# wendazhou/nbodyhpc

Hardware: AMD Instinct MI355X
Metric: kNN queries/sec (k=32, 1e8 periodic particles) (higher is better)
Workload: dtype f32; 1 GPU; kNN k=32 self-query of every particle, 1e+08 uniform periodic particles (L=1.0), leafsize 64; n_particles=100000000, n_particles_per_gpu=100000000, k=32, leafsize=64, parallelism=single

## Files before the change

### include/nbkd.h

```cpp
#ifndef NBKD_H
#define NBKD_H

#include <stdint.h>

#ifdef __cplusplus
extern "C" {
#endif

typedef int32_t nbkd_status;

enum {
    NBKD_OK = 0,
    NBKD_EINVAL = 1,
    NBKD_EBOX = 2,
    NBKD_ETOOMANY = 3,
    NBKD_ENOMEM = 4,
    NBKD_EDEVICE = 5,
    NBKD_EINTR = 6
};

#define NBKD_INPUT_DEVICE 0x1u
#define NBKD_OUTPUT_DEVICE 0x2u
#define NBKD_ACCUMULATE 0x4u
#define NBKD_SQUARED 0x8u
// ... 74 lines not shown
                               uint32_t flags, void *stream);

nbkd_status nbkd_group_potential(const nbkd_tree *tree,
                                 const uint64_t *offsets, const uint32_t *members,
                                 uint64_t ngroups, uint64_t nmembers,
                                 const float *mass, float eps, uint32_t max_members,
                                 float *out_phi, uint32_t *out_minpos,
                                 uint32_t flags, void *stream);

nbkd_status nbkd_query_ball_csr(const nbkd_tree *tree, const float *q, uint64_t m, float r,
                                uint64_t *out_offsets, uint32_t *out_idx, uint64_t capacity,
                                uint32_t flags, void *stream);

nbkd_status nbkd_tree_info(const nbkd_tree *tree, uint64_t *n8, uint64_t *nodes,
                           int32_t *periodic, float *box_size, int32_t *device);

nbkd_status nbkd_export(const nbkd_tree *tree, nbkd_node *nodes, float *x, float *y, float *z,
                        uint32_t *idx);

void nbkd_free(nbkd_tree *tree);

nbkd_status nbkd_set_tuning(const char *name, double value);
nbkd_status nbkd_get_tuning(const char *name, double *value);

typedef int (*nbkd_interrupt_fn)(void *user);
nbkd_status nbkd_set_interrupt(nbkd_interrupt_fn fn, void *user);

const char *nbkd_last_error(void);

nbkd_status nbkd_device_count(int32_t *count);

nbkd_status nbkd_timing_enable(int32_t enable);
nbkd_status nbkd_timing_reset(void);
nbkd_status nbkd_timing_read(const char *name, double *ms, uint64_t *launches);

nbkd_status nbkd_stats_enable(int32_t enable);
nbkd_status nbkd_stats_read(uint64_t *nodes_visited, uint64_t *points_scanned);
nbkd_status nbkd_stats_read_all(uint64_t *out, int32_t n);


nbkd_status nbkd_set_ids(nbkd_tree *tree, const uint32_t *ids, uint32_t flags, void *stream);

nbkd_status nbkd_set_kth_out(nbkd_tree *tree, float *kth, uint64_t capacity);

nbkd_status nbkd_slab_select(const float *xyz, const uint32_t *ids, uint64_t n, float lo, float hi,
                             float *out_xyz, uint32_t *out_ids, uint64_t capacity,
// ... 43 lines not shown
```

### nbodyhpc_amd/capi.py

```python
from __future__ import annotations

import ctypes
import os
import re

import numpy as np

PKG = os.path.dirname(os.path.abspath(__file__))
LIB_PATH = os.environ.get("NBKD_LIB") or os.path.join(PKG, "lib", "libnbkd.so")
HEADER = os.path.join(os.path.dirname(PKG), "include", "nbkd.h")

NBKD_OK, NBKD_EINVAL, NBKD_EBOX, NBKD_ETOOMANY, NBKD_ENOMEM, NBKD_EDEVICE, NBKD_EINTR = range(7)
NBKD_INPUT_DEVICE = 0x1
NBKD_OUTPUT_DEVICE = 0x2
NBKD_ACCUMULATE = 0x4
NBKD_SQUARED = 0x8
NBKD_SORTED = 0x10
KERNEL_TOPHAT, KERNEL_CUBIC, KERNEL_WENDLAND = 0, 1, 2
NBKD_MAX_VALUES = 4
NBKD_MAX_RADII = 32
NBKD_EWALD_N = 64

NODE_DTYPE = np.dtype([("dim", "<i4"), ("split", "<f4"), ("left", "<u4"), ("right", "<u4")])

# ... 44 lines not shown
    "nbkd_last_error": (ctypes.c_char_p, []),
    "nbkd_device_count": (_i32, [ctypes.POINTER(_i32)]),
    "nbkd_timing_enable": (_i32, [_i32]),
    "nbkd_timing_reset": (_i32, []),
    "nbkd_timing_read": (_i32, [ctypes.c_char_p, ctypes.POINTER(ctypes.c_double),
                                ctypes.POINTER(_u64)]),
    "nbkd_stats_enable": (_i32, [_i32]),
    "nbkd_stats_read": (_i32, [ctypes.POINTER(_u64), ctypes.POINTER(_u64)]),
    "nbkd_stats_read_all": (_i32, [ctypes.POINTER(_u64), _i32]),
    "nbkd_set_ids": (_i32, [_c_p, _c_p, _u32, _c_p]),
    "nbkd_slab_select": (_i32, [_c_p, _c_p, _u64, ctypes.c_float, ctypes.c_float, _c_p, _c_p,
                                _u64, ctypes.POINTER(_u64), _i32, _c_p]),
    "nbkd_slab_violations": (_i32, [_c_p, _c_p, _u64, _i32, ctypes.c_float, ctypes.c_float,
                                    ctypes.c_float, ctypes.POINTER(_u64), _i32, _c_p]),
    "nbkd_slab_forward": (_i32, [_c_p, _c_p, _u64, _i32, ctypes.c_float, ctypes.c_float, _c_p,
                                 _c_p, _u64, ctypes.POINTER(_u64), _i32, _c_p]),
    "nbkd_slab_forward_async": (_i32, [_c_p, _c_p, _u64, _i32, ctypes.c_float, ctypes.c_float,
                                       _c_p, _c_p, _u64, _c_p, _i32, _c_p]),
    "nbkd_rows_gather": (_i32, [_c_p, _u64, _c_p, _u64, _c_p, _i32, _c_p]),
    "nbkd_rows_scatter": (_i32, [_c_p, _u64, _c_p, _u64, _c_p, _i32, _c_p]),
    "nbkd_set_tuning": (_i32, [ctypes.c_char_p, ctypes.c_double]),
    "nbkd_set_interrupt": (_i32, [_c_p, _c_p]),
    "nbkd_get_tuning": (_i32, [ctypes.c_char_p, ctypes.POINTER(ctypes.c_double)]),
    "nbkd_comm_probe": (_i32, []),
    "nbkd_comm_unique_id": (_i32, [_c_p]),
    "nbkd_comm_init": (_i32, [_c_p, _i32, _i32, _i32, ctypes.POINTER(_c_p)]),
    "nbkd_comm_exchange": (_i32, [_c_p, _i32, _c_p, _c_p, _c_p, _c_p, _c_p, _c_p, _c_p]),
    "nbkd_comm_free": (None, [_c_p]),
    "nbkd_deposit": (_i32, [_c_p, _c_p, _c_p, _u64, _i32, _i32, _i32, ctypes.c_float, _c_p, _i32,
                            _i32, _i32, _i32, _c_p, _i32, _u32, _c_p]),
}
COMM_ID_BYTES = 128


def header_symbols() -> list[str]:
    txt = open(HEADER).read()
    txt = re.sub(r"/\*.*?\*/", "", txt, flags=re.S)
    return sorted(set(re.findall(r"\b(nbkd_[a-z_]+)\s*\(", txt)))


_lib = None


def lib():
    global _lib
    if _lib is None:
# ... 376 lines not shown
    flags = NBKD_INPUT_DEVICE | NBKD_OUTPUT_DEVICE | (NBKD_ACCUMULATE if accumulate else 0)
    _check(lib().nbkd_deposit(xyz_ptr, weight_ptr, radius_ptr, int(n), gx, gy, nz, float(ppu),
                              per.ctypes.data, int(subsample), int(mode), x0, wx, out_ptr,
                              int(device), flags, stream))


def ewald_table():
    nn = NBKD_EWALD_N + 1
    out = np.empty((nn, nn, nn, 4), np.float32)
    _check(lib().nbkd_ewald_table(out.ctypes.data, out.size))
    return out


def set_tuning(name, value):
    _check(lib().nbkd_set_tuning(name.encode(), float(value)))


def get_tuning(name):
    v = ctypes.c_double()
    _check(lib().nbkd_get_tuning(name.encode(), ctypes.byref(v)))
    return v.value


def timing_enable(on=True):
    _check(lib().nbkd_timing_enable(1 if on else 0))


def timing_reset():
    _check(lib().nbkd_timing_reset())


def timing_read(name):
    ms, cnt = ctypes.c_double(), _u64()
    _check(lib().nbkd_timing_read(name.encode(), ctypes.byref(ms), ctypes.byref(cnt)))
    return ms.value, cnt.value


def stats_enable(on=True):
    _check(lib().nbkd_stats_enable(1 if on else 0))


def stats_read():
    a, b = _u64(), _u64()
    _check(lib().nbkd_stats_read(ctypes.byref(a), ctypes.byref(b)))
    return a.value, b.value

# ... 100 lines not shown
```

### nbodyhpc_amd/csrc/api.cpp

```cpp
#include <hip/hip_runtime.h>

#include <sched.h>

#include <atomic>
#include <cmath>
#include <condition_variable>
#include <cstdio>
#include <cstring>
#include <map>
#include <mutex>
#include <new>
#include <string>
#include <thread>
#include <vector>

#include "internal.hpp"

namespace nbkd {

namespace {
thread_local std::string g_err;
thread_local uint64_t g_stats[NBKD_NSTATS] = {};

std::mutex g_tmu;
// ... 212 lines not shown
}

void tree_free(void *p) {
    if (!p) return;
    BlockCache &c = block_cache();
    std::lock_guard<std::mutex> g(c.mu);
    auto it = c.live.find(p);
    if (it == c.live.end()) {
        (void)hipFree(p);
        return;
    }
    const auto key = it->second;
    c.live.erase(it);
    if (c.idle_bytes + key.second <= BlockCache::CAP) {
        c.idle.insert({key, p});
        c.idle_bytes += key.second;
    } else {
        (void)hipFree(p);
    }
}


namespace {
std::atomic<double> g_tune[TUNE_N] = {{3.0}, {0.0}, {0.0}, {0.0}, {1.0}, {0.0}};
const char *const g_tune_names[TUNE_N] = {"knn_seed_margin", "candidate_bytes", "host_batch",
                                          "host_threads", "self_order", "pinned_bytes"};
thread_local nbkd_interrupt_fn t_intr = nullptr;
thread_local void *t_intr_user = nullptr;
}

double tuning(int id) { return g_tune[id].load(std::memory_order_relaxed); }

bool interrupted() { return t_intr != nullptr && t_intr(t_intr_user) != 0; }

Workspace &acquire_ws(const Tree &t) {
    if (t.ws.mu.try_lock()) return t.ws;
    {
        std::lock_guard<std::mutex> g(t.ws_mu);
        for (auto &w : t.ws_extra)
            if (w->mu.try_lock()) return *w;
        if ((int)t.ws_extra.size() < NBKD_MAX_WS - 1) {
            t.ws_extra.emplace_back(new Workspace());
            Workspace &w = *t.ws_extra.back();
            w.mu.lock();
            return w;
        }
    }
    t.ws.mu.lock();
    return t.ws;
// ... 703 lines not shown
    delete tree;
}

nbkd_status nbkd_set_tuning(const char *name, double value) {
    if (!name) {
        set_error("nbkd_set_tuning: NULL name");
        return NBKD_EINVAL;
    }
    for (int i = 0; i < TUNE_N; ++i) {
        if (std::strcmp(name, g_tune_names[i]) != 0) continue;
        const bool ok = i == TUNE_KNN_SEED ? (value > 0.0 && value <= 1e3)
                                           : (value >= 0.0 && value < 1e15);
        if (!ok || !std::isfinite(value)) {
            set_error(std::string("nbkd_set_tuning: value out of range for ") + name);
            return NBKD_EINVAL;
        }
        g_tune[i].store(value, std::memory_order_relaxed);
        return NBKD_OK;
    }
    set_error(std::string("nbkd_set_tuning: unknown knob ") + name);
    return NBKD_EINVAL;
}

nbkd_status nbkd_get_tuning(const char *name, double *value) {
    if (!name || !value) {
        set_error("nbkd_get_tuning: NULL argument");
        return NBKD_EINVAL;
    }
    for (int i = 0; i < TUNE_N; ++i)
        if (std::strcmp(name, g_tune_names[i]) == 0) {
            *value = tuning(i);
            return NBKD_OK;
        }
    set_error(std::string("nbkd_get_tuning: unknown knob ") + name);
    return NBKD_EINVAL;
}

nbkd_status nbkd_set_interrupt(nbkd_interrupt_fn fn, void *user) {
    t_intr = fn;
    t_intr_user = user;
    return NBKD_OK;
}

nbkd_status nbkd_timing_enable(int32_t enable) {
    g_timing = enable != 0;
    return NBKD_OK;
// ... 191 lines not shown
```

### nbodyhpc_amd/csrc/internal.hpp

```cpp
#pragma once

#include <hip/hip_runtime.h>

#include <cfloat>
#include <cstdint>
#include <cstdlib>
#include <memory>
#include <mutex>
#include <string>
#include <vector>

#include "../../include/nbkd.h"

namespace nbkd {

enum WsSlot {
    WS_Q = 0, WS_KEYS, WS_KEYS2, WS_ORDER, WS_TMP, WS_HIST, WS_SUMS, WS_OUTD, WS_OUTI,
    WS_COUNT, WS_OFF, WS_IDX, WS_STATS, WS_LIST, WS_LT, WS_TG, WS_CAND, WS_CCOUNT,
    WS_LIST2, WS_RSORT, WS_KTHD, WS_KTHI, WS_KB, WS_ANCH, WS_PAIR, WS_HTOT,
    WS_VT, WS_VALS, WS_HRAD,
    WS_GRAV,
    WS_HQ0, WS_HQ1, WS_HO00, WS_HO01, WS_HO10, WS_HO11, WS_NSLOTS
};
constexpr int NBKD_MAX_WS = 4;
// ... 116 lines not shown
    uint32_t n8;
    uint32_t nnodes;
    float box;
    const float *__restrict__ nbox;
};

inline DevTree view(const Tree &t) {
    return DevTree{t.x, t.y, t.z, t.idx, t.p4, t.nodes, (uint32_t)t.n8, (uint32_t)t.nnodes, t.box,
                   t.nbox};
}

#ifdef NBKD_EXPERIMENTS
inline const char *knob(const char *env) { return getenv(env); }
#else
inline const char *knob(const char *) { return nullptr; }
#endif
enum TuneId {
    TUNE_KNN_SEED = 0,
    TUNE_CAND_BYTES,
    TUNE_HOST_BATCH,
    TUNE_HOST_THREADS,
    TUNE_SELF_ORDER,
    TUNE_PINNED_BYTES,
    TUNE_N
};
void host_copy(void *dst, const void *src, size_t bytes);
int host_workers();
bool interrupted();
double tuning(int id);

void set_error(const std::string &msg);
nbkd_status hip_fail(hipError_t e, const char *what);

#define NBKD_HIP(call)                                                                     \
    do {                                                                                   \
        hipError_t e_ = (call);                                                            \
        if (e_ != hipSuccess) return ::nbkd::hip_fail(e_, #call);                          \
    } while (0)

struct TimedScope {
    TimedScope(const char *name, hipStream_t s, bool on = true);
    ~TimedScope();
    const char *name_;
    hipStream_t s_;
    hipEvent_t a_ = nullptr;
    int dev_ = 0;
// ... 33 lines not shown
nbkd_status build_tree(Tree &t, const float *xyz, uint64_t n, int32_t leaf_size, bool input_dev,
                       hipStream_t s);

struct QSpan {
    uint32_t m;
    const uint32_t *count;
    uint32_t base;
    uint32_t total;
    int mode;
    bool capped = false;
    bool tg_pos = false;
    uint32_t *out_list = nullptr;
    uint32_t *out_count = nullptr;
};
__host__ __device__ inline QSpan static_span(uint32_t m) { return QSpan{m, nullptr, 0u, 0u, 0}; }
__device__ __forceinline__ uint32_t span_m(const QSpan &s) {
    if (!s.count) return s.m;
    const uint32_t c = __builtin_amdgcn_readfirstlane(*s.count);
    if (s.mode != 0 && (((uint64_t)c * 512u >= (uint64_t)s.total) != (s.mode == 1))) return 0u;
    return c > s.base ? min(c - s.base, s.m) : 0u;
}

uint32_t collect_capacity(int k);
bool retry_adaptive();
nbkd_status launch_knn_collect(const Tree &t, const float *q, const uint32_t *order, QSpan span,
                               int k, const float *tg, float seed_mul, uint32_t qpp, uint2 *cand,
                               uint32_t capg, uint32_t *ccount, float *od, uint32_t *oi,
                               uint32_t *fail_list, uint32_t *fail_count, uint32_t *fail_bits,
                               uint32_t pos_base, bool retry, bool fix_seed, bool sq, float *kb,
                               unsigned long long *stats, hipStream_t s,
                               float *kth_side = nullptr, uint32_t *pair_scratch = nullptr);

nbkd_status launch_collect_pass(const Tree &t, const float *q, const uint32_t *order, QSpan span,
                                int k, const float *tg, float seed_mul, uint32_t qpp, uint2 *cand,
                                uint32_t capg, uint32_t *ccount, bool retry, float *kb,
                                unsigned long long *stats, hipStream_t s);
nbkd_status launch_select_pass(const Tree &t, const float *q, const uint32_t *order, QSpan span,
                               int k, const float *tg, uint32_t qpp, const uint2 *cand,
                               uint32_t capg, const uint32_t *ccount, float *od, uint32_t *oi,
                               uint32_t *fail_list, uint32_t *fail_count, uint32_t *fail_bits,
                               uint32_t pos_base, bool retry, bool fix_seed, bool sq, float *kb,
                               hipStream_t s, float *kth_side = nullptr,
                               uint32_t *pair_scratch = nullptr);

void launch_ball_packet(const Tree &t, const float *q, const uint32_t *order, uint32_t m, float r2,
                        uint32_t *out_count, const uint64_t *row_offsets, uint32_t *out_idx,
// ... 142 lines not shown
```

### nbodyhpc_amd/csrc/knn_collect.hip

```cpp
#include <algorithm>

#include "internal.hpp"
#include "metric.hpp"
#include "packet.hpp"

namespace nbkd {
namespace {
using namespace dev;

constexpr int TB = 256;
constexpr int WPB = TB / 64;

#ifndef NBKD_COL_ROWMAJOR
#define NBKD_COL_ROWMAJOR 1
#endif
#ifndef NBKD_PAIR_PAD
#define NBKD_PAIR_PAD 1
#endif
#ifndef NBKD_PAIR_ATOMIC
#define NBKD_PAIR_ATOMIC 1
#endif
#ifndef NBKD_SEL_FIRST
#define NBKD_SEL_FIRST 1
#endif
#ifndef NBKD_WAVE_KEY64
#define NBKD_WAVE_KEY64 1
#endif
#ifndef NBKD_WAVE_PAIR
#define NBKD_WAVE_PAIR 4
#endif
#ifndef NBKD_LOOP_AHEAD
#define NBKD_LOOP_AHEAD 1
#endif
#ifndef NBKD_RETRY_GROW
#define NBKD_RETRY_GROW 1.0f
#endif
#ifndef NBKD_RETRY_MINV
#define NBKD_RETRY_MINV 2.0f
#endif
#ifndef NBKD_SCL_EARLY
#define NBKD_SCL_EARLY 0
#endif
#ifndef NBKD_PAIR_PREFETCH
#define NBKD_PAIR_PREFETCH 0
#endif

constexpr int NB = 16;

__device__ __forceinline__ uint32_t d2_bucket(float d, float c) {
    return min((uint32_t)(d * c), (uint32_t)(NB - 1));
}


constexpr int GCHUNK = 64;
constexpr int GMAX = GCHUNK / NBKD_GROUP;

constexpr uint32_t PR_OWNER = NBKD_PAIR_PAD ? 7 : 6, PR_G = NBKD_PAIR_PAD ? 13 : 12;
constexpr uint32_t PR_SLOT = (1u << PR_OWNER) - 1u;
constexpr uint32_t PAIR_DUMMY = 64u;

struct CollectLdsG {
    float4 sq[64 + NBKD_PAIR_PAD];
    float scl[64];
    uint32_t cnt[64];
    uint32_t hist[NB / 4][65];
    float4 p4[GCHUNK];
    float gb[6 * GMAX];
    float tb[8];
    uint16_t pairs[64 * GMAX];
    uint8_t slot[64];
};

#define NBKD_COLLECT_STAGE_G(LPOS, CN, TBOX)                                                       \
    do {                                                                                           \
        glds_f4(t.p4 + (LPOS), W.p4, lane, (CN));                                                  \
        glds_f32(ginfo + 6 * (size_t)((LPOS) / NBKD_GROUP), W.gb, lane, 6 * ((CN) / NBKD_GROUP));  \
        glds_f32((TBOX), W.tb, lane, 6);                                                           \
    } while (0)

template <bool PER, bool M, bool STATS, bool AHEAD>
__device__ __forceinline__ void grp_packet(const DevTree &t, const float *__restrict__ ginfo,
                                           const uint32_t *__restrict__ linfo,
                                           const float *__restrict__ hinfo,
                                           CollectLdsG &W, const int lane, const float qx,
                                           const float qy, const float qz, float &kth,
                                           const float s_over_nb, const float nb_over_s,
                                           uint2 *__restrict__ col, const uint32_t qpp,
                                           const uint32_t capg, const int kq, uint32_t &cnt,
                                           uint32_t (&st)[13]) {
    const float L = t.box;
    uint32_t last_cnt = 0;
    const cnode_ptr cnodes = (cnode_ptr)t.nodes;
    const cbox_ptr cboxes = (cbox_ptr)t.nbox;
    PacketWalk wk;
    walk_begin(wk);
    uint64_t tclk = STATS ? clock64() : 0;
#define NBKD_PH(I)                                                                                 \
    do {                                                                                           \
        if constexpr (STATS) {                                                                     \
            const uint64_t t_ = clock64();                                                         \
            st[6 + (I)] += (uint32_t)(t_ - tclk);                                                              \
            tclk = t_;                                                                             \
        }                                                                                          \
    } while (0)
    bool ha = false;
    uint32_t pa = 0, ea = 0, lnode = 0;
    for (;;) {
        uint32_t pa_next = 0, ea_next = 0;
        const bool ha_next = walk_next_leaf<M, STATS>(wk, cnodes, cboxes, qx, qy, qz, kth, L, pa_next,
                                                      ea_next, st[0]);
        if constexpr (!AHEAD) {
            if (!ha_next) break;
            ha = true;
            pa = pa_next;
            ea = ea_next;
            lnode = wk.node;
        }
        if (ha) {
            const uint32_t lend = ea;
            const uint32_t lc = lend - pa;
            const bool halves = hinfo != nullptr && lc > (uint32_t)GCHUNK && lc <= 2u * GCHUNK;
            const uint32_t hm = (lc / 2) / 8 * 8;
            const float *const lbox = halves ? hinfo + 12 * (size_t)lnode
                                             : reinterpret_cast<const float *>(linfo) + 8 * (size_t)lnode;
            uint32_t c0 = pa;
            uint32_t cn = halves ? hm : min((uint32_t)GCHUNK, lc);
            if constexpr (!AHEAD) {
                if constexpr (STATS) ++st[3];
                NBKD_COLLECT_STAGE_G(pa, cn, lbox);
            }
            NBKD_PH(0);
            wait_vm0();
            wave_sync();
// ... 148 lines not shown
                wait_vm0();
                wave_sync();
            }
            wave_sync();
        }
        if constexpr (AHEAD) {
            if (!ha_next) break;
            ha = true;
            pa = pa_next;
            ea = ea_next;
            lnode = wk.node;
            if constexpr (STATS) ++st[3];
            const uint32_t lc = ea - pa;
            const bool halves = hinfo != nullptr && lc > (uint32_t)GCHUNK && lc <= 2u * GCHUNK;
            NBKD_COLLECT_STAGE_G(pa, halves ? (lc / 2) / 8 * 8 : min((uint32_t)GCHUNK, lc),
                                 halves ? hinfo + 12 * (size_t)lnode
                                        : reinterpret_cast<const float *>(linfo) + 8 * (size_t)lnode);
        }
    }
    NBKD_PH(0);
#undef NBKD_PH
}

template <bool PER, bool STATS, bool AHEAD>
__device__ __forceinline__ void collect_packet(
    const DevTree &t, const float *__restrict__ ginfo, const uint32_t *__restrict__ linfo,
    const float *__restrict__ hinfo, const float *__restrict__ q, const uint32_t *__restrict__ order,
    uint32_t m, int kq, const float *__restrict__ tg, bool tg_pos, float seed_mul, uint32_t qpp,
    uint2 *__restrict__ cand, uint32_t capg, uint32_t *__restrict__ ccount,
    unsigned long long *__restrict__ stats, float *__restrict__ kbound, CollectLdsG &W, int lane,
    uint32_t pk, uint32_t *__restrict__ out_list, uint32_t *__restrict__ out_count) {
    const uint32_t gq = pk * qpp + lane;
    const bool valid = (uint32_t)lane < qpp && gq < m;
    const uint32_t qo = valid ? order[gq] : 0u;
    const float qx = valid ? q[3 * (size_t)qo] : 0.0f;
    const float qy = valid ? q[3 * (size_t)qo + 1] : 0.0f;
    const float qz = valid ? q[3 * (size_t)qo + 2] : 0.0f;
    if constexpr (PER) {
        if (out_list && valid &&
            !(qx >= 0.0f && qx <= t.box && qy >= 0.0f && qy <= t.box && qz >= 0.0f && qz <= t.box))
            out_list[atomicAdd(out_count, 1u)] = qo;
    }
    const float seed = valid ? fminf(tg[tg_pos ? gq : qo] * seed_mul, FLT_MAX) : -INFINITY;
    const bool fin = seed < FLT_MAX && seed >= 1e-30f;
    const float s_over_nb = fin ? seed * (1.0f / NB) : (seed > 0.0f ? INFINITY : 0.0f);
    const float nb_over_s = fin ? (float)NB / seed * 1.00000095367431640625f : 0.0f;
#pragma unroll
    for (int w = 0; w < NB / 4; ++w) W.hist[w][lane] = 0u;
#if NBKD_PAIR_PAD
    if (lane == 0) W.sq[PAIR_DUMMY] = make_float4(0.0f, 0.0f, 0.0f, -INFINITY);
#endif
    uint2 *const col = cand + (size_t)pk * qpp * capg;
    uint32_t cnt = 0;
    uint32_t st[13] = {0, 0, 0, 0, 0, 0, 0, 0, 0, 0, 0, 0, 0};
    float kth = seed;
    bool plain = false;
    if constexpr (PER) {
        const float r1 = sqrtf(fmaxf(seed, 0.0f)) * 1.01f + t.box * 1e-6f;
        const bool wf = !valid || (fin && r1 <= 0.25f * t.box && qx >= r1 && t.box - qx >= r1 &&
                                   qy >= r1 && t.box - qy >= r1 && qz >= r1 && t.box - qz >= r1);
        plain = __all(wf);
    }
    if (plain)
        grp_packet<PER, false, STATS, AHEAD>(t, ginfo, linfo, hinfo, W, lane, qx, qy, qz, kth,
                                             s_over_nb, nb_over_s, col, qpp, capg, kq, cnt, st);
    else
        grp_packet<PER, PER, STATS, AHEAD>(t, ginfo, linfo, hinfo, W, lane, qx, qy, qz, kth,
                                           s_over_nb, nb_over_s, col, qpp, capg, kq, cnt, st);
    if (valid) ccount[gq] = cnt;
    if (valid && kbound) kbound[gq] = kth;
    if (STATS && lane == 0) {
        atomicAdd(&stats[0], (unsigned long long)st[0]);
        atomicAdd(&stats[1], (unsigned long long)st[5]);
        atomicAdd(&stats[2], (unsigned long long)st[3]);
        atomicAdd(&stats[3], (unsigned long long)st[4]);
        atomicAdd(&stats[4], (unsigned long long)st[2]);
        atomicAdd(&stats[5], 1ull);
        atomicAdd(&stats[7], (unsigned long long)st[1]);
#pragma unroll
        for (int i = 0; i < 6; ++i) atomicAdd(&stats[10 + i], (unsigned long long)st[6 + i]);
        atomicAdd(&stats[16], (unsigned long long)st[12]);
    }
    if (STATS) {
        uint32_t c = valid ? cnt : 0u;
#pragma unroll
        for (int o = 32; o > 0; o >>= 1) c += __shfl_xor(c, o, 64);
        if (lane == 0) atomicAdd(&stats[6], (unsigned long long)c);
    }
}

template <bool PER, int OCC, bool STATS, bool LOOP, bool AHEAD>
__global__ void __launch_bounds__(TB, OCC)
knn_collect_grp_kernel(DevTree t, const float *__restrict__ ginfo,
                       const uint32_t *__restrict__ linfo, const float *__restrict__ hinfo,
                       const float *__restrict__ q,
                       const uint32_t *__restrict__ order, QSpan span, int kq,
                       const float *__restrict__ tg, float seed_mul, uint32_t qpp,
                       uint2 *__restrict__ cand, uint32_t capg,
                       uint32_t *__restrict__ ccount, unsigned long long *__restrict__ stats,
                       bool xcd, float *__restrict__ kbound) {
    __shared__ CollectLdsG Wl[WPB];
    const int lane = threadIdx.x & 63, wave = wave_id();
    CollectLdsG &W = Wl[wave];
    const uint32_t m = span_m(span);
    const uint32_t npk = (m + qpp - 1) / qpp;
    const uint32_t bid = xcd ? xcd_block(blockIdx.x, gridDim.x) : blockIdx.x;
    if constexpr (LOOP) {
        for (uint32_t pk = bid * WPB + wave; pk < npk; pk += gridDim.x * WPB) {
            wave_sync();
            collect_packet<PER, STATS, AHEAD>(t, ginfo, linfo, hinfo, q, order, m, kq, tg, span.tg_pos,
                                              seed_mul, qpp, cand, capg, ccount, stats, kbound,
                                              W, lane, pk, span.out_list, span.out_count);
        }
    } else {
        const uint32_t pk = bid * WPB + wave;
        if (pk < npk)
            collect_packet<PER, STATS, AHEAD>(t, ginfo, linfo, hinfo, q, order, m, kq, tg, span.tg_pos,
                                              seed_mul, qpp, cand, capg, ccount, stats, kbound,
                                              W, lane, pk, span.out_list, span.out_count);
    }
}

template <bool PER>
__device__ __forceinline__ void mark_failure(float qx, float qy, float qz, float L, uint32_t id,
                                             uint32_t *fail_list, uint32_t *fail_count,
                                             uint32_t *fail_bits) {
    if (PER && !(qx >= 0.0f && qx <= L && qy >= 0.0f && qy <= L && qz >= 0.0f && qz <= L)) return;
    if (fail_bits)
        atomicOr(&fail_bits[id >> 5], 1u << (id & 31u));
    else
        fail_list[atomicAdd(fail_count, 1u)] = id;
}

__device__ __forceinline__ void issue_block(const uint4 *b4, uint4 *lds4, int lane, uint64_t rows,
                                            uint32_t row_stride4) {
    const uint32_t r0 = (uint32_t)lane >> 3, jj = (uint32_t)lane & 7u;
    const uint4 *src = b4 + r0 * row_stride4 + (jj ^ r0);
    const uint32_t m = (uint32_t)((((rows >> r0) & 0x0101010101010101ull) * 0x0102040810204080ull) >> 56);
#pragma unroll
    for (int i = 0; i < 8; ++i)
// ... 556 lines not shown
        return 8u * (unsigned)std::max(cus, 1);
    }();
    return b;
}

template <bool PER>
void launch_collect(const Tree &t, const float *q, const uint32_t *order, QSpan span, int k,
                    const float *tg, float seed_mul, uint32_t qpp, uint2 *cand, uint32_t capg,
                    uint32_t *ccount, unsigned long long *stats, bool retry, float *kbound,
                    hipStream_t s) {
    const char *const name = retry ? "knn_retry" : "knn_collect";
    const uint32_t m = span.m;
    const unsigned blocks =
        span.count ? std::min<unsigned>(resident_blocks(),
                                        (unsigned)((((uint64_t)m + qpp - 1) / qpp + WPB - 1) / WPB))
                   : (unsigned)((((uint64_t)m + qpp - 1) / qpp + WPB - 1) / WPB);
    if (k > 255) k = 0x7FFFFFFF;
    {
        static const bool xcd = [] {
            const char *e = knob("NBKD_XCD_MAP");
            return !(e && atoi(e) == 0);
        }();
        TimedScope ts(name, s, !retry);
#define NBKD_GRP(STATS, LOOP, AHEAD, STP, XCD)                                                     \
    knn_collect_grp_kernel<PER, 8, STATS, LOOP, AHEAD><<<blocks, TB, 0, s>>>(                      \
        view(t), t.ginfo, t.leafinfo, t.hinfo, q, order, span, k, tg, seed_mul, qpp, cand, capg,   \
        ccount, STP, XCD, kbound)
        if (span.count)
            NBKD_GRP(false, true, NBKD_LOOP_AHEAD != 0, nullptr, false);
        else if (collect_ahead()) {
            if (stats)
                NBKD_GRP(true, false, true, stats, xcd);
            else
                NBKD_GRP(false, false, true, nullptr, xcd);
        } else if (stats)
            NBKD_GRP(true, false, false, stats, xcd);
        else
            NBKD_GRP(false, false, false, nullptr, xcd);
#undef NBKD_GRP
        return;
    }
}

template <int R>
void launch_select_wave(const Tree &t, const float *q, const uint32_t *order, QSpan span, int k,
                        uint32_t qpp, const uint2 *cand, uint32_t capg, const uint32_t *ccount,
                        float *od, uint32_t *oi, uint32_t *fail_list, uint32_t *fail_count,
                        uint32_t *fail_bits, uint32_t pos_base, float *tg_fix, float mu, bool sq,
                        const float *kbound, hipStream_t s, uint32_t *pair_scratch) {
    const uint32_t *pos_list = nullptr;
    if constexpr (R == 2 && NBKD_COL_ROWMAJOR && NBKD_WAVE_PAIR > 0) {
        if (pair_scratch && !span.count && kbound) {
            uint32_t *nleft = pair_scratch + ((size_t)span.m + 15) / 16 * 16;
            if (hipMemsetAsync(nleft, 0, 4, s) != hipSuccess) goto one_query;
            {
            constexpr int NQ = NBKD_WAVE_PAIR;
            const unsigned pblocks = (unsigned)std::min<uint64_t>(
                (((uint64_t)span.m + NQ - 1) / NQ + WPB - 1) / WPB, 32768u);
            if (t.periodic)
                knn_select_wave_pair_kernel<true, NQ><<<pblocks, TB, 0, s>>>(
                    order, span, k, cand, capg, ccount, od, oi, sq, kbound, pair_scratch, nleft);
            else
// ... 48 lines not shown
        if (t.periodic) {
            if (qpp == 64) NBKD_SELECT(true, true, true); else NBKD_SELECT(true, false, true);
        } else {
            if (qpp == 64) NBKD_SELECT(false, true, true); else NBKD_SELECT(false, false, true);
        }
    } else {
        if (t.periodic) {
            if (qpp == 64) NBKD_SELECT(true, true, false); else NBKD_SELECT(true, false, false);
        } else {
            if (qpp == 64) NBKD_SELECT(false, true, false); else NBKD_SELECT(false, false, false);
        }
    }
#undef NBKD_SELECT
}

}

bool retry_adaptive() {
    static const bool on = [] {
        const char *e = knob("NBKD_RETRY_ADAPT");
        return !(e && atoi(e) == 0);
    }();
    return on;
}

uint32_t collect_capacity(int k) {
    const double mu = k + 4.0 * std::sqrt((double)k) + 4.0;
    double c = mu + 5.0 * std::sqrt(mu);
    if (const char *e = knob("NBKD_KNN_CAP")) c *= std::max(0.25, atof(e));
    return (uint32_t)((c + 15.0) / 16.0) * 16u;
}

nbkd_status launch_knn_collect(const Tree &t, const float *q, const uint32_t *order, QSpan span,
                               int k, const float *tg, float seed_mul, uint32_t qpp, uint2 *cand,
                               uint32_t capg, uint32_t *ccount, float *od, uint32_t *oi,
                               uint32_t *fail_list, uint32_t *fail_count, uint32_t *fail_bits,
                               uint32_t pos_base, bool retry, bool fix_seed, bool sq, float *kb,
                               unsigned long long *stats, hipStream_t s, float *kth_side,
                               uint32_t *pair_scratch) {
    nbkd_status rc = launch_collect_pass(t, q, order, span, k, tg, seed_mul, qpp, cand, capg,
                                         ccount, retry, kb, stats, s);
    if (rc) return rc;
    return launch_select_pass(t, q, order, span, k, tg, qpp, cand, capg, ccount, od, oi,
                              fail_list, fail_count, fail_bits, pos_base, retry, fix_seed, sq, kb,
                              s, kth_side, pair_scratch);
}
// ... 61 lines not shown
```

### nbodyhpc_amd/csrc/packet.hpp

```cpp
#pragma once

#include "metric.hpp"

namespace nbkd {
namespace dev {

typedef __attribute__((address_space(1))) const void *gas_ptr;
typedef __attribute__((address_space(3))) void *las_ptr;

__device__ __forceinline__ void glds_f32(const float *src, float *dst, int lane, uint32_t n) {
    if ((uint32_t)lane < n)
        __builtin_amdgcn_global_load_lds((gas_ptr)(src + lane), (las_ptr)dst, 4, 0, 0);
}

__device__ __forceinline__ void glds_f4(const float4 *src, float4 *dst, int lane, uint32_t n) {
    if ((uint32_t)lane < n)
        __builtin_amdgcn_global_load_lds((gas_ptr)(src + lane), (las_ptr)dst, 16, 0, 0);
}

__device__ __forceinline__ void wait_vm0() { __builtin_amdgcn_s_waitcnt(0x0F70); }

constexpr int pow2_floor(int v) { return v >= 64 ? 64 : v >= 32 ? 32 : v >= 16 ? 16 : v >= 8 ? 8 : 4; }
constexpr int pow2_ceil(int v) { return v <= 4 ? 4 : v <= 8 ? 8 : v <= 16 ? 16 : v <= 32 ? 32 : 64; }

// ... 150 lines not shown
        else                                                                                       \
            NBKD_GSTEP(2)                                                                          \
    }


struct PacketWalk {
    uint32_t node;
    int sp;
    uint32_t sk_node;
    uint32_t bx[6];
    float tm[3];
};

__device__ __forceinline__ void walk_begin(PacketWalk &w) {
    w.node = 0;
    w.sp = 1;
    w.sk_node = 0;
#pragma unroll
    for (int a = 0; a < 6; ++a) w.bx[a] = 0u;
#pragma unroll
    for (int a = 0; a < 3; ++a) w.tm[a] = 0.0f;
}

template <bool M>
__device__ __forceinline__ bool walk_step(PacketWalk &w, const int D, const uint32_t split_bits,
                                          const uint32_t left, const uint32_t right, uint64_t &wm,
                                          const float qx, const float qy, const float qz,
                                          const float kth, const float L) {
    const float split = __uint_as_float(split_bits);
    const float qd = D == 0 ? qx : (D == 1 ? qy : qz);
    float tl, tr;
    if constexpr (M) {
        const uint32_t lo = D == 0 ? w.bx[0] : (D == 1 ? w.bx[2] : w.bx[4]);
        const uint32_t hi = D == 0 ? w.bx[1] : (D == 1 ? w.bx[3] : w.bx[5]);
        tl = box_lb_axis<M>(qd, __uint_as_float(lo), split, L);
        tr = box_lb_axis<M>(qd, split, __uint_as_float(hi), L);
    } else {
        const float tmd = D == 0 ? w.tm[0] : (D == 1 ? w.tm[1] : w.tm[2]);
        const float dd = qd - split;
        const float m2 = dd * dd;
        tl = dd > 0.0f ? m2 : tmd;
        tr = dd > 0.0f ? tmd : m2;
    }
    const float dl = ((D == 0 ? tl : w.tm[0]) + (D == 1 ? tl : w.tm[1])) + (D == 2 ? tl : w.tm[2]);
    const float dr = ((D == 0 ? tr : w.tm[0]) + (D == 1 ? tr : w.tm[1])) + (D == 2 ? tr : w.tm[2]);
    const uint64_t wl = __ballot(dl <= kth), wr = __ballot(dr <= kth);
    bool go_right = wr != 0;
    if (wl != 0 && wr != 0) {
        const uint32_t right_votes = (uint32_t)__popcll(wm & __ballot(qd > split));
        go_right = 2 * right_votes > (uint32_t)__popcll(wm);
        w.sk_node = lane_set(w.sk_node, go_right ? left : right, 1ull << w.sp);
        ++w.sp;
    }
    w.node = go_right ? right : left;
    const float tn = go_right ? tr : tl;
    w.tm[0] = D == 0 ? tn : w.tm[0];
    w.tm[1] = D == 1 ? tn : w.tm[1];
    w.tm[2] = D == 2 ? tn : w.tm[2];
#pragma unroll
    for (int a = 0; a < 3; ++a) {
        w.bx[2 * a] = (D == a && go_right) ? split_bits : w.bx[2 * a];
        w.bx[2 * a + 1] = (D == a && !go_right) ? split_bits : w.bx[2 * a + 1];
    }
    wm = go_right ? wr : wl;
    return (wl | wr) != 0;
}

template <bool M, bool STATS>
__device__ __forceinline__ bool walk_next_leaf(PacketWalk &w, const cnode_ptr cnodes,
                                               const cbox_ptr cboxes, const float qx,
                                               const float qy, const float qz, const float kth,
                                               const float L, uint32_t &lpos, uint32_t &lend,
                                               uint32_t &visits) {
    enum : int { RUN = 0, LEAF = 1, DONE = 2 };
    bool loaded = false;
    int end = RUN;
    int dim = 0;
    uint32_t split_bits = 0, left = 0, right = 0;
    uint64_t wm = 0;
    do {
        if (!loaded) {
            if (w.sp == 0) {
                end = DONE;
            } else {
                --w.sp;
                w.node = (uint32_t)__builtin_amdgcn_readlane((int)w.sk_node, w.sp);
                const NodeBox nb = cboxes[w.node];
                const nbkd_node nd = cnodes[w.node];
#pragma unroll
                for (int a = 0; a < 6; ++a) w.bx[a] = uni(__float_as_uint(nb.b[a]));
                dim = (int)uni((uint32_t)nd.dimension);
                split_bits = uni(__float_as_uint(nd.split));
                left = uni(nd.left);
                right = uni(nd.right);
                w.tm[0] = box_lb_axis<M>(qx, __uint_as_float(w.bx[0]), __uint_as_float(w.bx[1]), L);
                w.tm[1] = box_lb_axis<M>(qy, __uint_as_float(w.bx[2]), __uint_as_float(w.bx[3]), L);
                w.tm[2] = box_lb_axis<M>(qz, __uint_as_float(w.bx[4]), __uint_as_float(w.bx[5]), L);
                wm = __ballot((w.tm[0] + w.tm[1]) + w.tm[2] <= kth);
                loaded = wm != 0;
            }
        }
        if (loaded) {
            if constexpr (STATS) ++visits;
            if (dim < 0) {
                lpos = left;
                lend = right;
                end = LEAF;
            } else {
                if (dim == 0)
                    loaded = walk_step<M>(w, 0, split_bits, left, right, wm, qx, qy, qz, kth, L);
                else if (dim == 1)
                    loaded = walk_step<M>(w, 1, split_bits, left, right, wm, qx, qy, qz, kth, L);
                else
                    loaded = walk_step<M>(w, 2, split_bits, left, right, wm, qx, qy, qz, kth, L);
                const nbkd_node nd = cnodes[w.node];
                dim = (int)uni((uint32_t)nd.dimension);
                split_bits = uni(__float_as_uint(nd.split));
                left = uni(nd.left);
                right = uni(nd.right);
            }
        }
    } while (end == RUN);
    return end == LEAF;
}

}
}
```

Baseline: 2.003 billion queries/s.

## Add inline-asm scalar tree descent and 32-bit node addressing for kNN walk

Adds a narrow-address path that indexes node and box arrays with 32-bit byte offsets through the constant address space, and a hand-written inline assembly descent loop that keeps the current node in fixed SGPRs, loads each child with s_load_dwordx4 and makes branch decisions on scalar masks. The aim is to shorten the per-node dependency chain of the packet walk, covering address arithmetic, readfirstlane moves and compiler-generated branching. It is on by default for non-periodic-crossing packets when the node count fits, and can be switched off with a tuning knob. Hardcoded SGPRs s68–s71 in the assembly carry a risk of register-allocation conflicts, and the assembly adds maintenance burden.

```diff
diff --git a/include/nbkd.h b/include/nbkd.h
--- a/include/nbkd.h
+++ b/include/nbkd.h
@@ -120,6 +120,7 @@
 
 nbkd_status nbkd_set_tuning(const char *name, double value);
 nbkd_status nbkd_get_tuning(const char *name, double *value);
+int32_t nbkd_collect_wide_addr(uint64_t nodes);
 
 typedef int (*nbkd_interrupt_fn)(void *user);
 nbkd_status nbkd_set_interrupt(nbkd_interrupt_fn fn, void *user);
diff --git a/nbodyhpc_amd/capi.py b/nbodyhpc_amd/capi.py
--- a/nbodyhpc_amd/capi.py
+++ b/nbodyhpc_amd/capi.py
@@ -90,6 +90,7 @@
     "nbkd_set_tuning": (_i32, [ctypes.c_char_p, ctypes.c_double]),
     "nbkd_set_interrupt": (_i32, [_c_p, _c_p]),
     "nbkd_get_tuning": (_i32, [ctypes.c_char_p, ctypes.POINTER(ctypes.c_double)]),
+    "nbkd_collect_wide_addr": (_i32, [_u64]),
     "nbkd_comm_probe": (_i32, []),
     "nbkd_comm_unique_id": (_i32, [_c_p]),
     "nbkd_comm_init": (_i32, [_c_p, _i32, _i32, _i32, ctypes.POINTER(_c_p)]),
@@ -512,6 +513,10 @@
     return v.value
 
 
+def collect_wide_addr(nodes):
+    return bool(lib().nbkd_collect_wide_addr(int(nodes)))
+
+
 def timing_enable(on=True):
     _check(lib().nbkd_timing_enable(1 if on else 0))
 
diff --git a/nbodyhpc_amd/csrc/api.cpp b/nbodyhpc_amd/csrc/api.cpp
--- a/nbodyhpc_amd/csrc/api.cpp
+++ b/nbodyhpc_amd/csrc/api.cpp
@@ -258,9 +258,10 @@
 
 
 namespace {
-std::atomic<double> g_tune[TUNE_N] = {{3.0}, {0.0}, {0.0}, {0.0}, {1.0}, {0.0}};
+std::atomic<double> g_tune[TUNE_N] = {{3.0}, {0.0}, {0.0}, {0.0}, {1.0}, {0.0}, {0.0}};
 const char *const g_tune_names[TUNE_N] = {"knn_seed_margin", "candidate_bytes", "host_batch",
-                                          "host_threads", "self_order", "pinned_bytes"};
+                                          "host_threads", "self_order", "pinned_bytes",
+                                          "collect_wide_addr"};
 thread_local nbkd_interrupt_fn t_intr = nullptr;
 thread_local void *t_intr_user = nullptr;
 }
@@ -1010,6 +1011,8 @@
     return NBKD_EINVAL;
 }
 
+int32_t nbkd_collect_wide_addr(uint64_t nodes) { return collect_wide_addr(nodes) ? 1 : 0; }
+
 nbkd_status nbkd_get_tuning(const char *name, double *value) {
     if (!name || !value) {
         set_error("nbkd_get_tuning: NULL argument");
diff --git a/nbodyhpc_amd/csrc/internal.hpp b/nbodyhpc_amd/csrc/internal.hpp
--- a/nbodyhpc_amd/csrc/internal.hpp
+++ b/nbodyhpc_amd/csrc/internal.hpp
@@ -162,6 +162,7 @@
     TUNE_HOST_THREADS,
     TUNE_SELF_ORDER,
     TUNE_PINNED_BYTES,
+    TUNE_COLLECT_WIDE,
     TUNE_N
 };
 void host_copy(void *dst, const void *src, size_t bytes);
@@ -241,6 +242,7 @@
 }
 
 uint32_t collect_capacity(int k);
+bool collect_wide_addr(uint64_t nnodes);
 bool retry_adaptive();
 nbkd_status launch_knn_collect(const Tree &t, const float *q, const uint32_t *order, QSpan span,
                                int k, const float *tg, float seed_mul, uint32_t qpp, uint2 *cand,
diff --git a/nbodyhpc_amd/csrc/knn_collect.hip b/nbodyhpc_amd/csrc/knn_collect.hip
--- a/nbodyhpc_amd/csrc/knn_collect.hip
+++ b/nbodyhpc_amd/csrc/knn_collect.hip
@@ -40,6 +40,9 @@
 #endif
 #ifndef NBKD_SCL_EARLY
 #define NBKD_SCL_EARLY 0
+#endif
+#ifndef NBKD_WALK_ASM
+#define NBKD_WALK_ASM 1
 #endif
 #ifndef NBKD_PAIR_PREFETCH
 #define NBKD_PAIR_PREFETCH 0
@@ -78,7 +81,7 @@
         glds_f32((TBOX), W.tb, lane, 6);                                                           \
     } while (0)
 
-template <bool PER, bool M, bool STATS, bool AHEAD>
+template <bool PER, bool M, bool STATS, bool AHEAD, bool NARROW>
 __device__ __forceinline__ void grp_packet(const DevTree &t, const float *__restrict__ ginfo,
                                            const uint32_t *__restrict__ linfo,
                                            const float *__restrict__ hinfo,
@@ -107,8 +110,13 @@
     uint32_t pa = 0, ea = 0, lnode = 0;
     for (;;) {
         uint32_t pa_next = 0, ea_next = 0;
-        const bool ha_next = walk_next_leaf<M, STATS>(wk, cnodes, cboxes, qx, qy, qz, kth, L, pa_next,
-                                                      ea_next, st[0]);
+        bool ha_next;
+        if constexpr (NBKD_WALK_ASM != 0 && !M && NARROW)
+            ha_next = walk_next_leaf_plain<STATS>(wk, cnodes, cboxes, qx, qy, qz, kth, L, pa_next,
+                                                  ea_next, st[0]);
+        else
+            ha_next = walk_next_leaf<M, STATS, NARROW>(wk, cnodes, cboxes, qx, qy, qz, kth, L,
+                                                       pa_next, ea_next, st[0]);
         if constexpr (!AHEAD) {
             if (!ha_next) break;
             ha = true;
@@ -303,7 +311,7 @@
 #undef NBKD_PH
 }
 
-template <bool PER, bool STATS, bool AHEAD>
+template <bool PER, bool STATS, bool AHEAD, bool NARROW>
 __device__ __forceinline__ void collect_packet(
     const DevTree &t, const float *__restrict__ ginfo, const uint32_t *__restrict__ linfo,
     const float *__restrict__ hinfo, const float *__restrict__ q, const uint32_t *__restrict__ order,
@@ -343,10 +351,10 @@
         plain = __all(wf);
     }
     if (plain)
-        grp_packet<PER, false, STATS, AHEAD>(t, ginfo, linfo, hinfo, W, lane, qx, qy, qz, kth,
+        grp_packet<PER, false, STATS, AHEAD, NARROW>(t, ginfo, linfo, hinfo, W, lane, qx, qy, qz, kth,
                                              s_over_nb, nb_over_s, col, qpp, capg, kq, cnt, st);
     else
-        grp_packet<PER, PER, STATS, AHEAD>(t, ginfo, linfo, hinfo, W, lane, qx, qy, qz, kth,
+        grp_packet<PER, PER, STATS, AHEAD, NARROW>(t, ginfo, linfo, hinfo, W, lane, qx, qy, qz, kth,
                                            s_over_nb, nb_over_s, col, qpp, capg, kq, cnt, st);
     if (valid) ccount[gq] = cnt;
     if (valid && kbound) kbound[gq] = kth;
@@ -370,7 +378,7 @@
     }
 }
 
-template <bool PER, int OCC, bool STATS, bool LOOP, bool AHEAD>
+template <bool PER, int OCC, bool STATS, bool LOOP, bool AHEAD, bool NARROW>
 __global__ void __launch_bounds__(TB, OCC)
 knn_collect_grp_kernel(DevTree t, const float *__restrict__ ginfo,
                        const uint32_t *__restrict__ linfo, const float *__restrict__ hinfo,
@@ -389,14 +397,14 @@
     if constexpr (LOOP) {
         for (uint32_t pk = bid * WPB + wave; pk < npk; pk += gridDim.x * WPB) {
             wave_sync();
-            collect_packet<PER, STATS, AHEAD>(t, ginfo, linfo, hinfo, q, order, m, kq, tg, span.tg_pos,
+            collect_packet<PER, STATS, AHEAD, NARROW>(t, ginfo, linfo, hinfo, q, order, m, kq, tg, span.tg_pos,
                                               seed_mul, qpp, cand, capg, ccount, stats, kbound,
                                               W, lane, pk, span.out_list, span.out_count);
         }
     } else {
         const uint32_t pk = bid * WPB + wave;
         if (pk < npk)
-            collect_packet<PER, STATS, AHEAD>(t, ginfo, linfo, hinfo, q, order, m, kq, tg, span.tg_pos,
+            collect_packet<PER, STATS, AHEAD, NARROW>(t, ginfo, linfo, hinfo, q, order, m, kq, tg, span.tg_pos,
                                               seed_mul, qpp, cand, capg, ccount, stats, kbound,
                                               W, lane, pk, span.out_list, span.out_count);
     }
@@ -999,10 +1007,18 @@
             return !(e && atoi(e) == 0);
         }();
         TimedScope ts(name, s, !retry);
-#define NBKD_GRP(STATS, LOOP, AHEAD, STP, XCD)                                                     \
-    knn_collect_grp_kernel<PER, 8, STATS, LOOP, AHEAD><<<blocks, TB, 0, s>>>(                      \
+        const bool narrow = !collect_wide_addr((uint64_t)t.nnodes);
+#define NBKD_GRP_(STATS, LOOP, AHEAD, STP, XCD, NARROW)                                            \
+    knn_collect_grp_kernel<PER, 8, STATS, LOOP, AHEAD, NARROW><<<blocks, TB, 0, s>>>(              \
         view(t), t.ginfo, t.leafinfo, t.hinfo, q, order, span, k, tg, seed_mul, qpp, cand, capg,   \
         ccount, STP, XCD, kbound)
+#define NBKD_GRP(STATS, LOOP, AHEAD, STP, XCD)                                                     \
+    do {                                                                                           \
+        if (narrow)                                                                                \
+            NBKD_GRP_(STATS, LOOP, AHEAD, STP, XCD, true);                                         \
+        else                                                                                       \
+            NBKD_GRP_(STATS, LOOP, AHEAD, STP, XCD, false);                                        \
+    } while (0)
         if (span.count)
             NBKD_GRP(false, true, NBKD_LOOP_AHEAD != 0, nullptr, false);
         else if (collect_ahead()) {
@@ -1015,6 +1031,7 @@
         else
             NBKD_GRP(false, false, false, nullptr, xcd);
 #undef NBKD_GRP
+#undef NBKD_GRP_
         return;
     }
 }
@@ -1109,6 +1126,10 @@
         return !(e && atoi(e) == 0);
     }();
     return on;
+}
+
+bool collect_wide_addr(uint64_t nnodes) {
+    return !dev::walk_narrow_ok(nnodes) || tuning(TUNE_COLLECT_WIDE) != 0.0;
 }
 
 uint32_t collect_capacity(int k) {
diff --git a/nbodyhpc_amd/csrc/packet.hpp b/nbodyhpc_amd/csrc/packet.hpp
--- a/nbodyhpc_amd/csrc/packet.hpp
+++ b/nbodyhpc_amd/csrc/packet.hpp
@@ -196,6 +196,30 @@
     for (int a = 0; a < 3; ++a) w.tm[a] = 0.0f;
 }
 
+#if defined(__HIP_DEVICE_COMPILE__)
+typedef const __attribute__((address_space(4))) char *cbyte_ptr;
+#else
+typedef const char *cbyte_ptr;
+#endif
+template <bool NARROW>
+__device__ __forceinline__ nbkd_node walk_load_node(const cnode_ptr cnodes, const uint32_t id) {
+    if constexpr (NARROW)
+        return *reinterpret_cast<cnode_ptr>(reinterpret_cast<cbyte_ptr>(cnodes) +
+                                            id * (uint32_t)sizeof(nbkd_node));
+    else
+        return cnodes[id];
+}
+template <bool NARROW>
+__device__ __forceinline__ NodeBox walk_load_box(const cbox_ptr cboxes, const uint32_t id) {
+    if constexpr (NARROW)
+        return *reinterpret_cast<cbox_ptr>(reinterpret_cast<cbyte_ptr>(cboxes) +
+                                           id * (uint32_t)sizeof(NodeBox));
+    else
+        return cboxes[id];
+}
+constexpr uint64_t WALK_NARROW_NODES = (1ull << 32) / sizeof(NodeBox);
+inline bool walk_narrow_ok(uint64_t nnodes) { return nnodes < WALK_NARROW_NODES; }
+
 template <bool M>
 __device__ __forceinline__ bool walk_step(PacketWalk &w, const int D, const uint32_t split_bits,
                                           const uint32_t left, const uint32_t right, uint64_t &wm,
@@ -240,7 +264,7 @@
     return (wl | wr) != 0;
 }
 
-template <bool M, bool STATS>
+template <bool M, bool STATS, bool NARROW>
 __device__ __forceinline__ bool walk_next_leaf(PacketWalk &w, const cnode_ptr cnodes,
                                                const cbox_ptr cboxes, const float qx,
                                                const float qy, const float qz, const float kth,
@@ -259,8 +283,8 @@
             } else {
                 --w.sp;
                 w.node = (uint32_t)__builtin_amdgcn_readlane((int)w.sk_node, w.sp);
-                const NodeBox nb = cboxes[w.node];
-                const nbkd_node nd = cnodes[w.node];
+                const NodeBox nb = walk_load_box<NARROW>(cboxes, w.node);
+                const nbkd_node nd = walk_load_node<NARROW>(cnodes, w.node);
 #pragma unroll
                 for (int a = 0; a < 6; ++a) w.bx[a] = uni(__float_as_uint(nb.b[a]));
                 dim = (int)uni((uint32_t)nd.dimension);
@@ -287,7 +311,7 @@
                     loaded = walk_step<M>(w, 1, split_bits, left, right, wm, qx, qy, qz, kth, L);
                 else
                     loaded = walk_step<M>(w, 2, split_bits, left, right, wm, qx, qy, qz, kth, L);
-                const nbkd_node nd = cnodes[w.node];
+                const nbkd_node nd = walk_load_node<NARROW>(cnodes, w.node);
                 dim = (int)uni((uint32_t)nd.dimension);
                 split_bits = uni(__float_as_uint(nd.split));
                 left = uni(nd.left);
@@ -298,5 +322,166 @@
     return end == LEAF;
 }
 
-}
-}
+#define NBKD_WD_AXIS(Q, TM, A, B)                                                                  \
+    "v_subrev_f32_e32 %[a], s69, " Q "\n"                                                          \
+    "v_cmp_lt_f32_e32 vcc, 0, %[a]\n"                                                              \
+    "v_mul_f32_e32 %[b], %[a], %[a]\n"                                                             \
+    "s_nop 0\n"                                                                                    \
+    "v_cndmask_b32_e32 %[c], " TM ", %[b], vcc\n"                                                  \
+    "v_cndmask_b32_e32 %[b], %[b], " TM ", vcc\n"                                                  \
+    "v_add_f32_e32 %[a], %[c], " A "\n"                                                            \
+    "v_add_f32_e32 %[d], %[b], " A "\n"                                                            \
+    "v_add_f32_e32 %[a], %[a], " B "\n"                                                            \
+    "v_add_f32_e32 %[d], %[d], " B "\n"                                                            \
+    "v_cmp_le_f32_e64 %[wl], %[a], %[kth]\n"                                                       \
+    "v_cmp_le_f32_e64 %[wr], %[d], %[kth]\n"
+#define NBKD_WD_AXIS2(Q, TM, A, B)                                                                 \
+    "v_subrev_f32_e32 %[a], s69, " Q "\n"                                                          \
+    "v_cmp_lt_f32_e32 vcc, 0, %[a]\n"                                                              \
+    "v_mul_f32_e32 %[b], %[a], %[a]\n"                                                             \
+    "v_add_f32_e32 %[d], " A ", " B "\n"                                                           \
+    "v_cndmask_b32_e32 %[c], " TM ", %[b], vcc\n"                                                  \
+    "v_cndmask_b32_e32 %[b], %[b], " TM ", vcc\n"                                                  \
+    "v_add_f32_e32 %[a], %[d], %[c]\n"                                                             \
+    "v_add_f32_e32 %[d], %[d], %[b]\n"                                                             \
+    "v_cmp_le_f32_e64 %[wl], %[a], %[kth]\n"                                                       \
+    "v_cmp_le_f32_e64 %[wr], %[d], %[kth]\n"
+#define NBKD_WD_DECIDE(T, Q, TM)                                                                   \
+    "s_cmp_lg_u64 %[wr], 0\n"                                                                      \
+    "s_cbranch_scc0 .Lwd_" T "nr_%=\n"                                                             \
+    "s_cmp_lg_u64 %[wl], 0\n"                                                                      \
+    "s_cbranch_scc0 .Lwd_" T "R_%=\n"                                                              \
+    "v_cmp_lt_f32_e32 vcc, s69, " Q "\n"                                                           \
+    "s_and_b64 vcc, vcc, %[wm]\n"                                                                  \
+    "s_bcnt1_i32_b64 %[s0], vcc\n"                                                                 \
+    "s_bcnt1_i32_b64 %[s1], %[wm]\n"                                                               \
+    "s_lshl_b32 %[s0], %[s0], 1\n"                                                                 \
+    "s_lshl_b64 %[pm], 1, %[sp]\n"                                                                 \
+    "s_add_i32 %[sp], %[sp], 1\n"                                                                  \
+    "s_cmp_gt_u32 %[s0], %[s1]\n"                                                                  \
+    "s_cbranch_scc1 .Lwd_" T "pR_%=\n"                                                             \
+    "v_mov_b32_e32 %[a], s71\n"                                                                    \
+    "v_cndmask_b32_e64 %[sk], %[sk], %[a], %[pm]\n"                                                \
+    ".Lwd_" T "L_%=:\n"                                                                            \
+    "v_mov_b32_e32 " TM ", %[c]\n"                                                                 \
+    "s_mov_b64 %[wm], %[wl]\n"                                                                     \
+    "s_mov_b32 %[nd], s70\n"                                                                       \
+    "s_branch .Lwd_load_%=\n"                                                                      \
+    ".Lwd_" T "nr_%=:\n"                                                                           \
+    "s_cmp_lg_u64 %[wl], 0\n"                                                                      \
+    "s_cbranch_scc1 .Lwd_" T "L_%=\n"                                                              \
+    "s_branch .Lwd_none_%=\n"                                                                      \
+    ".Lwd_" T "pR_%=:\n"                                                                           \
+    "v_mov_b32_e32 %[a], s70\n"                                                                    \
+    "v_cndmask_b32_e64 %[sk], %[sk], %[a], %[pm]\n"                                                \
+    ".Lwd_" T "R_%=:\n"                                                                            \
+    "v_mov_b32_e32 " TM ", %[b]\n"                                                                 \
+    "s_mov_b64 %[wm], %[wr]\n"                                                                     \
+    "s_mov_b32 %[nd], s71\n"
+#define NBKD_WD_BODY(VISIT)                                                                        \
+    "s_mov_b32 s68, %[dim]\n"                                                                      \
+    "s_mov_b32 s69, %[spl]\n"                                                                      \
+    "s_mov_b32 s70, %[lf]\n"                                                                       \
+    "s_mov_b32 s71, %[rt]\n"                                                                       \
+    ".Lwd_top_%=:\n" VISIT                                                                         \
+    "s_cmp_lt_i32 s68, 0\n"                                                                        \
+    "s_cbranch_scc1 .Lwd_leaf_%=\n"                                                                \
+    "s_cmp_eq_u32 s68, 1\n"                                                                        \
+    "s_cbranch_scc1 .Lwd_y_%=\n"                                                                   \
+    "s_cmp_eq_u32 s68, 0\n"                                                                        \
+    "s_cbranch_scc1 .Lwd_x_%=\n"                                                                   \
+    NBKD_WD_AXIS2("%[qz]", "%[tm2]", "%[tm0]", "%[tm1]")                                           \
+    NBKD_WD_DECIDE("z", "%[qz]", "%[tm2]")                                                         \
+    "s_branch .Lwd_load_%=\n"                                                                      \
+    ".Lwd_y_%=:\n"                                                                                 \
+    NBKD_WD_AXIS("%[qy]", "%[tm1]", "%[tm0]", "%[tm2]")                                            \
+    NBKD_WD_DECIDE("y", "%[qy]", "%[tm1]")                                                         \
+    "s_branch .Lwd_load_%=\n"                                                                      \
+    ".Lwd_x_%=:\n"                                                                                 \
+    NBKD_WD_AXIS("%[qx]", "%[tm0]", "%[tm1]", "%[tm2]")                                            \
+    NBKD_WD_DECIDE("x", "%[qx]", "%[tm0]")                                                         \
+    ".Lwd_load_%=:\n"                                                                              \
+    "s_lshl_b32 %[s0], %[nd], 4\n"                                                                 \
+    "s_load_dwordx4 s[68:71], %[base], %[s0] offset:0x0\n"                                         \
+    "s_waitcnt lgkmcnt(0)\n"                                                                       \
+    "s_branch .Lwd_top_%=\n"                                                                       \
+    ".Lwd_none_%=:\n"                                                                              \
+    "s_mov_b32 %[dim], 0\n"                                                                        \
+    "s_branch .Lwd_end_%=\n"                                                                       \
+    ".Lwd_leaf_%=:\n"                                                                              \
+    "s_mov_b32 %[dim], s68\n"                                                                      \
+    "s_mov_b32 %[lf], s70\n"                                                                       \
+    "s_mov_b32 %[rt], s71\n"                                                                       \
+    ".Lwd_end_%=:\n"
+#define NBKD_WD_OPERANDS                                                                           \
+    [dim] "+s"(dim), [lf] "+s"(left), [rt] "+s"(right), [nd] "+s"(w.node), [sp] "+s"(w.sp),        \
+        [wm] "+s"(wm), [tm0] "+v"(w.tm[0]), [tm1] "+v"(w.tm[1]), [tm2] "+v"(w.tm[2]),              \
+        [sk] "+v"(w.sk_node), [a] "=&v"(ta), [b] "=&v"(tb), [c] "=&v"(tc), [d] "=&v"(td),          \
+        [wl] "=&s"(wl), [wr] "=&s"(wr), [pm] "=&s"(pm), [s0] "=&s"(s0), [s1] "=&s"(s1)
+template <bool STATS>
+__device__ __forceinline__ void walk_descend(PacketWalk &w, const cnode_ptr cnodes, uint32_t &dim,
+                                             const uint32_t split_bits, uint32_t &left,
+                                             uint32_t &right, uint64_t wm, const float qx,
+                                             const float qy, const float qz, const float kth,
+                                             uint32_t &visits) {
+    float ta, tb, tc, td;
+    uint64_t wl, wr, pm;
+    uint32_t s0, s1;
+    const uint64_t base = (uint64_t)cnodes;
+    if constexpr (STATS)
+        asm volatile(NBKD_WD_BODY("s_add_u32 %[vis], %[vis], 1\n")
+                     : NBKD_WD_OPERANDS, [vis] "+s"(visits)
+                     : [spl] "s"(split_bits), [base] "s"(base), [qx] "v"(qx), [qy] "v"(qy),
+                       [qz] "v"(qz), [kth] "v"(kth)
+                     : "s68", "s69", "s70", "s71", "vcc", "scc");
+    else
+        asm volatile(NBKD_WD_BODY("")
+                     : NBKD_WD_OPERANDS
+                     : [spl] "s"(split_bits), [base] "s"(base), [qx] "v"(qx), [qy] "v"(qy),
+                       [qz] "v"(qz), [kth] "v"(kth)
+                     : "s68", "s69", "s70", "s71", "vcc", "scc");
+}
+#undef NBKD_WD_OPERANDS
+#undef NBKD_WD_BODY
+#undef NBKD_WD_DECIDE
+#undef NBKD_WD_AXIS2
+#undef NBKD_WD_AXIS
+
+template <bool STATS>
+__device__ __forceinline__ bool walk_next_leaf_plain(PacketWalk &w, const cnode_ptr cnodes,
+                                                     const cbox_ptr cboxes, const float qx,
+                                                     const float qy, const float qz,
+                                                     const float kth, const float L,
+                                                     uint32_t &lpos, uint32_t &lend,
+                                                     uint32_t &visits) {
+    uint32_t found = 0, dim = 0, left = 0, right = 0;
+    while (w.sp != 0) {
+        --w.sp;
+        w.node = (uint32_t)__builtin_amdgcn_readlane((int)w.sk_node, w.sp);
+        const NodeBox nb = walk_load_box<true>(cboxes, w.node);
+        const nbkd_node nd = walk_load_node<true>(cnodes, w.node);
+#pragma unroll
+        for (int a = 0; a < 6; ++a) w.bx[a] = uni(__float_as_uint(nb.b[a]));
+        dim = uni((uint32_t)nd.dimension);
+        const uint32_t split_bits = uni(__float_as_uint(nd.split));
+        left = uni(nd.left);
+        right = uni(nd.right);
+        w.tm[0] = box_lb_axis<false>(qx, __uint_as_float(w.bx[0]), __uint_as_float(w.bx[1]), L);
+        w.tm[1] = box_lb_axis<false>(qy, __uint_as_float(w.bx[2]), __uint_as_float(w.bx[3]), L);
+        w.tm[2] = box_lb_axis<false>(qz, __uint_as_float(w.bx[4]), __uint_as_float(w.bx[5]), L);
+        const uint64_t wm = __ballot((w.tm[0] + w.tm[1]) + w.tm[2] <= kth);
+        if (wm == 0) continue;
+        walk_descend<STATS>(w, cnodes, dim, split_bits, left, right, wm, qx, qy, qz, kth, visits);
+        if ((int)dim < 0) {
+            asm volatile("");
+            found = 1;
+            break;
+        }
+    }
+    lpos = left;
+    lend = right;
+    return found != 0;
+}
+
+}
+}
```

Result: faster. 2.086 billion queries/s, median of 6 (+4.2%).
